# ZhonghuaYi/EI-Nexus_official

Measured on AMD Instinct MI355X. Metric: event-image pairs/s (extract+match, 346x260, 1024 kpts), higher is better.
Workload: dtype f32; 1 GPU; B32 346x260 5-bin event voxel + gray image, VGG(event)+SuperPoint(image) extractors, MNN matcher, k=1024; global_batch=32, event_bins=5, parallelism=dp1 (pairs sharded, metric all-reduce only), log_assignment=False, dense_outputs=False, same_scene_pairs=False, weights=seeded synthetic, descriptor-head bias calibrated (per-channel mean removed)

## Files before the change

### ei-nexus_official_amd/_lib.py

```python
import ctypes
import os

_HERE = os.path.dirname(os.path.abspath(__file__))
LIB_PATH = os.environ.get("EINX_LIB") or os.path.join(_HERE, "libeinx_hip.so")

c_void_p, c_int, c_float, c_size_t, c_char_p = ctypes.c_void_p, ctypes.c_int, ctypes.c_float, ctypes.c_size_t, ctypes.c_char_p


class ConvDesc(ctypes.Structure):
    _fields_ = [("w_native", c_void_p), ("bias", c_void_p), ("scale", c_void_p), ("shift", c_void_p),
                ("cin", ctypes.c_int32), ("cout", ctypes.c_int32), ("ks", ctypes.c_int32), ("relu", ctypes.c_int32),
                ("pool", ctypes.c_int32)]


class DetectParams(ctypes.Structure):
    _fields_ = [("B", ctypes.c_int32), ("Hp", ctypes.c_int32), ("Wp", ctypes.c_int32), ("H", ctypes.c_int32),
                ("W", ctypes.c_int32), ("h0", ctypes.c_int32), ("w0", ctypes.c_int32), ("radius", ctypes.c_int32),
                ("top_k", ctypes.c_int32), ("det_thr", c_float), ("ordering_xy", ctypes.c_int32), ("cap", ctypes.c_int32),
                ("nms_iters", ctypes.c_int32)]


class ExtractorDesc(ctypes.Structure):
    _fields_ = [("struct_size", c_size_t), ("cell", ctypes.c_int32), ("n_backbone", ctypes.c_int32), ("n_det", ctypes.c_int32), ("n_desc", ctypes.c_int32),
                ("backbone", ctypes.POINTER(ConvDesc)), ("det_head", ctypes.POINTER(ConvDesc)), ("desc_head", ctypes.POINTER(ConvDesc)),
# ... 41 lines not shown
                ("t_type", ctypes.c_int32), ("p_type", ctypes.c_int32), ("n", ctypes.c_int64)]


class LgLayer(ctypes.Structure):
    _names = ("Wqkv", "bqkv", "Wo", "bo", "sf0_w", "sf0_b", "sln_g", "sln_b", "sf3_w", "sf3_b",
              "Wqk", "bqk", "Wv", "bv", "Wco", "bco", "cf0_w", "cf0_b", "cln_g", "cln_b", "cf3_w", "cf3_b", "Wqk_v", "bqk_v")
    _fields_ = [(n, c_void_p) for n in _names]


class LgWeights(ctypes.Structure):
    _fields_ = [("struct_size", c_size_t), ("layer_size", c_size_t), ("in_w", c_void_p), ("in_b", c_void_p), ("Wr", c_void_p), ("proj_w", c_void_p), ("proj_b", c_void_p),
                ("match_w", c_void_p), ("match_b", c_void_p), ("n_layers", ctypes.c_int32), ("heads", ctypes.c_int32),
                ("d", ctypes.c_int32), ("input_dim", ctypes.c_int32), ("filter_threshold", c_float),
                ("layers", ctypes.POINTER(LgLayer))]


class LgHead(ctypes.Structure):
    _fields_ = [(n, c_void_p) for n in ("proj_w", "proj_b", "match_w", "match_b", "token_w", "token_b")]


SIGNATURES = {
    "einx_version": (c_char_p, []),
    "einx_abi_version": (c_int, []),
    "einx_build_flags": (c_char_p, []),
    "einx_params_hash": (c_int, [c_void_p, c_int, c_void_p, c_void_p, c_void_p, c_void_p]),
    "einx_last_error": (c_char_p, []),
    "einx_math_eval": (c_int, [c_int, c_void_p, ctypes.c_longlong, c_void_p, c_void_p]),
    "einx_fork_stream_of": (c_void_p, [c_void_p]),
    "einx_fork_stream_prepare_beside": (c_int, [c_void_p, ctypes.POINTER(c_void_p), c_int]),
    "einx_stream_overlap_us": (c_int, [c_void_p, c_void_p, c_int, ctypes.POINTER(ctypes.c_float)]),
    "einx_device_count": (c_int, []),
    "einx_profile_enable": (c_int, [c_int]),
    "einx_profile_report": (c_int, [c_char_p, c_size_t]),
    "einx_extractor_create": (c_void_p, [ctypes.POINTER(ExtractorDesc)]),
    "einx_extractor_destroy": (None, [c_void_p]),
    "einx_fork_stream_prepare": (c_int, [c_void_p]),
    "einx_fork_stream_release": (c_int, [c_void_p]),
    "einx_fork_stream_count": (c_int, []),
    "einx_side_stream": (c_void_p, [c_void_p, c_int, ctypes.POINTER(c_void_p), c_int]),
    "einx_extract_shapes": (c_int, [c_void_p, c_int, c_int, ctypes.POINTER(ExtractShapes)]),
    "einx_extract_ws_bytes": (c_size_t, [c_void_p, c_int, c_int, c_int, c_int, c_int]),
    "einx_extract": (c_int, [c_void_p, c_void_p, c_void_p, c_int, c_int, c_int, c_int, c_void_p, c_size_t, ctypes.POINTER(ExtractOut), c_void_p]),
    "einx_extract_watch": (c_int, [c_void_p, c_void_p, c_void_p, c_int, c_int, c_int, c_int, c_void_p, c_size_t, ctypes.POINTER(ExtractOut),
                           ctypes.POINTER(WeightWatch), c_void_p]),
    "einx_conv_last_kernel": (c_char_p, []),
    "einx_conv_plan": (c_char_p, [c_int] * 11),
    "einx_conv_weight_elems": (c_size_t, [c_int, c_int, c_int]),
    "einx_conv_repack": (c_int, [c_void_p, c_int, c_int, c_int, c_void_p, c_void_p]),
    "einx_bn_fold": (c_int, [c_void_p, c_void_p, c_void_p, c_void_p, c_float, c_int, c_void_p, c_void_p, c_void_p]),
    "einx_conv_block": (c_int, [c_void_p, c_int, c_int, c_int, c_int, c_int, c_int, c_int, ctypes.POINTER(ConvDesc), c_void_p, c_void_p]),
    "einx_conv_first_two_fused_ok": (c_int, [ctypes.POINTER(ConvDesc), ctypes.POINTER(ConvDesc), c_int, c_int, c_int]),
    "einx_conv_first_two_fused": (c_int, [c_void_p, c_int, c_int, c_int, c_int, c_int, c_int, c_int, ctypes.POINTER(ConvDesc), ctypes.POINTER(ConvDesc),
                                  c_void_p, c_void_p]),
    "einx_div_inplace": (c_int, [c_void_p, c_size_t, c_float, c_void_p]),
    "einx_image_prepare": (c_int, [c_void_p, c_int, c_int, c_int, c_int, ctypes.c_longlong, ctypes.c_longlong, ctypes.c_longlong, ctypes.c_longlong,
                           c_float, c_void_p, c_void_p]),
    "einx_score_map": (c_int, [c_void_p, c_int, c_int, c_int, c_int, c_void_p, c_int, c_int, c_int, c_int, c_int, c_int, c_void_p,
                               c_void_p, c_void_p]),
    "einx_remove_border": (c_int, [c_void_p, c_int, c_int, c_int, c_int, c_void_p]),
    "einx_detect_ws_bytes": (c_size_t, [ctypes.POINTER(DetectParams)]),
    "einx_detect": (c_int, [c_void_p, ctypes.POINTER(DetectParams), c_void_p, c_void_p, c_void_p, c_void_p, c_void_p, c_void_p,
                            c_void_p, c_void_p]),
    "einx_desc_sample": (c_int, [c_void_p, c_int, c_int, c_int, c_int, c_int, c_int, c_int, c_int, c_void_p, c_void_p, c_int, c_float,
                                 c_void_p, c_void_p]),
    "einx_normalize_map": (c_int, [c_void_p, c_int, c_int, c_int, c_float, c_void_p, c_void_p, c_void_p]),
    "einx_upsample_ws_bytes": (c_size_t, [c_int, c_int, c_int]),
    "einx_upsample_normalize": (c_int, [c_void_p, c_int, c_int, c_int, c_int, c_int, c_int, c_int, c_int, c_int, c_int, c_float,
                                        c_void_p, c_void_p, c_size_t, c_void_p]),
    "einx_mnn_ws_bytes": (c_size_t, [c_int, c_int, c_int]),
    "einx_mnn": (c_int, [c_void_p, c_void_p, c_int, c_void_p, c_void_p, c_int, c_int, c_int, c_void_p, c_void_p, c_void_p, c_void_p,
                         c_void_p, c_void_p, c_void_p]),
    "einx_mnn_gather": (c_int, [c_void_p, c_void_p, c_int, c_void_p, c_void_p, c_int, c_int, c_int, c_void_p, c_void_p, c_void_p, c_void_p,
                                c_void_p, c_void_p, c_void_p, c_void_p, c_int, c_void_p, c_void_p, c_void_p, c_void_p]),
    "einx_mnn_thresh": (c_int, [c_void_p, c_void_p, c_int, c_void_p, c_void_p, c_int, c_int, c_int, c_int, c_float, c_int, c_float, c_void_p,
                                c_void_p, c_void_p, c_void_p, c_void_p, c_void_p, c_void_p]),
    "einx_gather_matches": (c_int, [c_void_p, c_void_p, c_void_p, c_void_p, c_int, c_int, c_int, c_int, c_void_p, c_void_p, c_void_p,
                                    c_void_p]),
    "einx_events_ws_bytes": (c_size_t, [c_int, c_int, c_int]),
    "einx_voxel_ws_bytes": (c_size_t, [c_int, c_int, c_int, c_int, ctypes.c_int64]),
    "einx_voxel_grid": (c_int, [c_void_p, c_void_p, c_void_p, c_void_p, c_void_p, c_int, c_int, c_int, c_int, c_int, c_void_p, c_void_p,
                                c_size_t, c_void_p]),
    "einx_events_mask": (c_int, [c_void_p, c_void_p, c_void_p, c_int, c_int, c_int, c_void_p, c_void_p, c_void_p]),
    "einx_time_surface_ws_bytes": (c_size_t, [c_int, c_int, c_int, c_int, ctypes.c_int64]),
    "einx_event_stack_ws_bytes": (c_size_t, [c_int, c_int, c_int, c_int, ctypes.c_int64]),
    "einx_distance_map_ws_bytes": (c_size_t, [c_int, c_int, c_int, c_int, ctypes.c_int64]),
    "einx_time_surface": (c_int, [c_void_p, c_void_p, c_void_p, c_void_p, c_void_p, c_int, c_int, c_int, c_int, c_void_p, c_void_p, c_size_t,
                                  c_void_p]),
    "einx_event_stack": (c_int, [c_void_p, c_void_p, c_void_p, c_void_p, c_void_p, c_int, c_int, c_int, c_int, c_void_p, c_void_p, c_size_t,
                                 c_void_p]),
    "einx_distance_map": (c_int, [c_void_p, c_void_p, c_void_p, c_void_p, c_void_p, c_int, c_int, c_int, c_int, c_void_p, c_void_p, c_size_t,
                                  c_void_p]),
    "einx_distance_map_plan": (c_char_p, [c_int, c_int]),
    "einx_events_windows_ws_bytes": (c_size_t, [c_int, c_int, c_int]),
    "einx_voxel_windows_ws_bytes": (c_size_t, [c_int, c_int, c_int, c_int, ctypes.c_int64]),
    "einx_voxel_grid_windows": (c_int, [c_void_p, c_void_p, c_void_p, c_void_p, ctypes.c_int64, c_void_p, c_void_p, c_int, c_int, c_int, c_int, c_int,
                                        c_void_p, c_void_p, c_size_t, c_void_p]),
    "einx_events_mask_windows": (c_int, [c_void_p, c_void_p, ctypes.c_int64, c_void_p, c_void_p, c_int, c_int, c_int, c_void_p, c_size_t, c_void_p,
                                         c_void_p]),
    "einx_events_pack": (c_int, [ctypes.POINTER(EventArrays), c_int, c_void_p, c_void_p, c_void_p, c_void_p, c_void_p, c_int]),
    "einx_metrics_ws_bytes": (c_size_t, [ctypes.POINTER(MetricParams)]),
    "einx_pair_metrics": (c_int, [ctypes.POINTER(MetricParams)] + [c_void_p] * 13),
    "einx_relative_pose_ws_bytes": (c_size_t, [ctypes.POINTER(PoseParams)]),
    "einx_relative_pose": (c_int, [ctypes.POINTER(PoseParams)] + [c_void_p] * 13),
    "einx_essential_5pt": (c_int, [c_void_p, c_void_p, c_int, c_void_p, c_void_p, c_void_p]),
    "einx_homography_ws_bytes": (c_size_t, [ctypes.POINTER(HomographyParams)]),
    "einx_homography": (c_int, [ctypes.POINTER(HomographyParams)] + [c_void_p] * 11),
# ... 67 lines not shown
```

### ei-nexus_official_amd/csrc/conv.hip

```cpp
#include <stdio.h>
#include <stdlib.h>

#include <type_traits>

#include "einx_common.h"

namespace {

constexpr int kCoutTile = 64;

struct ConvArgs {
  const float* in;
  const float* w;
  const float* bias;
  const float* scale;
  const float* shift;
  float* out;
  int B, Cin, Cout, CoutPad;
  int Hs, Ws, h0, w0;
  int H, W;
  int tilesX, tilesY;
  int relu;
};

// ... 819 lines not shown
    const float* ib = in_b + (size_t)c * CK * HW;
#pragma unroll
    for (int i = 0; i < IN_PER_THR; ++i) r_in[i] = ib[goff[i]];
    const float* wb = a.w + (size_t)c * CK * a.CoutPad;
#pragma unroll
    for (int i = 0; i < W_PER_THR; ++i) r_w[i] = *reinterpret_cast<const f32x4*>(wb + woff[i]);
  };
  f32x4v acc[NPW];
#pragma unroll
  for (int n = 0; n < NPW; ++n) acc[n] = f32x4v{0.0f, 0.0f, 0.0f, 0.0f};
  const int nchunks = a.Cin / CK;
  issue_loads(0);
  float e_bi[4], e_sc[4], e_sh[4];
#pragma unroll
  for (int i = 0; i < 4; ++i) {
    const int coc = min(co0 + wave * 16 + 4 * q + i, a.Cout - 1);
    e_bi[i] = a.bias ? a.bias[coc] : 0.0f;
    e_sc[i] = a.scale ? a.scale[coc] : 1.0f;
    e_sh[i] = a.scale ? a.shift[coc] : 0.0f;
  }
  const int aoff = q * WP + wave * 16 + j, boff = q * NPX + j;
  for (int c = 0; c < nchunks; ++c) {
    __syncthreads();
#pragma unroll
    for (int i = 0; i < IN_PER_THR; ++i) in_tile[loff[i]] = r_in[i];
#pragma unroll
    for (int i = 0; i < W_PER_THR; ++i) *reinterpret_cast<f32x4*>(w_tile + wl[i]) = r_w[i];
    __syncthreads();
    if (c + 1 < nchunks) issue_loads(c + 1);
    float av[G], bv[G][NPW];
#pragma unroll
    for (int g = 0; g < G; ++g) {
      av[g] = w_tile[aoff + g * 4 * WP];
#pragma unroll
      for (int n = 0; n < NPW; ++n) bv[g][n] = in_tile[boff + g * 4 * NPX + 16 * n];
    }
#pragma unroll
    for (int g = 0; g < G; ++g)
#pragma unroll
      for (int n = 0; n < NPW; ++n) acc[n] = __builtin_amdgcn_mfma_f32_16x16x4f32(av[g], bv[g][n], acc[n], 0, 0, 0);
  }
  float* out_b = a.out + (size_t)b * a.Cout * HW;
#pragma unroll
  for (int i = 0; i < 4; ++i) {
    const int co = co0 + wave * 16 + 4 * q + i;
#pragma unroll
    for (int n = 0; n < NPW; ++n) {
      const int p = p0 + 16 * n + j;
      float v = acc[n][i] + e_bi[i];
      if (a.relu) v = v > 0.0f ? v : 0.0f;
      if (a.scale) v = fmaf(v, e_sc[i], e_sh[i]);
      if (co < a.Cout && p < HW) out_b[(size_t)co * HW + p] = v;
    }
  }
}

__global__ void conv_repack_kernel(const float* w, int cin, int cout, int taps, int coutPad, int krows, float* out) {
  const size_t n = (size_t)krows * coutPad;
  for (size_t i = (size_t)blockIdx.x * blockDim.x + threadIdx.x; i < n; i += (size_t)gridDim.x * blockDim.x) {
    const int co = (int)(i % coutPad);
    const int k = (int)(i / coutPad);
    const int h = k & 1;
    const int tap = (k >> 1) % taps;
    const int cp = (k >> 1) / taps;
    const int ci = 2 * cp + h;
    float v = 0.0f;
    if (ci < cin && co < cout) v = w[((size_t)co * cin + ci) * taps + tap];
    out[i] = v;
  }
}

__global__ void bn_fold_kernel(const float* g, const float* b, const float* mean, const float* var, float eps, int n, float* scale,
                               float* shift) {
  const int i = blockIdx.x * blockDim.x + threadIdx.x;
  if (i >= n) return;
  const float s = g[i] / sqrtf(var[i] + eps);
  scale[i] = s;
  shift[i] = b[i] - mean[i] * s;
}

int native_krows(int cin, int taps) { return einx_cdiv(cin, 32) * 32 * taps; }

thread_local const char* g_last_conv_kernel = "";

struct TileCfg {
  int th, tw, slots;
};

template <int KS, int TH, int TW, int WM, int WN, int MT, int NT, int CK, bool POOL, bool DENSE3 = false>
void launch(const ConvArgs& a, int B, hipStream_t s, bool three_per_cu = false) {
  dim3 grid((unsigned)(a.tilesX * a.tilesY * B), (unsigned)(a.CoutPad / kCoutTile));
  const bool three = DENSE3 && three_per_cu;
  {
    static char nm[2][96] = {{0}, {0}};
    char* n = nm[three ? 1 : 0];
    if (!n[0]) snprintf(n, sizeof nm[0], "conv_block_kernel<%d,%d,%d,%d,%d,%d,%d,%d,%s>%s", KS, TH, TW, WM, WN, MT, NT, CK, POOL ? "true" : "false", three ? " (3 per CU)" : "");
    g_last_conv_kernel = n;
  }
  EINX_PROF(KS == 1 ? "conv_block_kernel 1x1" : (CK < 8 ? "conv_block_kernel 3x3 first layer" : "conv_block_kernel 3x3"), s);
  if constexpr (DENSE3) {
    if (three) {
      hipLaunchKernelGGL((conv_block_kernel<KS, TH, TW, WM, WN, MT, NT, CK, POOL, false, 6>), grid, dim3(WM * WN * 64), 0, s, a);
      return;
    }
  }
  hipLaunchKernelGGL((conv_block_kernel<KS, TH, TW, WM, WN, MT, NT, CK, POOL>), grid, dim3(WM * WN * 64), 0, s, a);
// ... 336 lines not shown
    EINX_CONV_BLOCK_VARIANTS(X)
#undef X
    case CB_1X1_128_XTRA: {
      dim3 grid((unsigned)(a.tilesX * B), (unsigned)(a.CoutPad / kCoutTile - 1));
      conv_plan_name(p, d->pool, nm, sizeof nm);
      g_last_conv_kernel = nm;
      EINX_PROF("conv_block_kernel 1x1", s);
      hipLaunchKernelGGL((conv_block_kernel<1, 1, 128, 1, 4, 2, 1, 32, false, true>), grid, dim3(256), 0, s, a);
      break;
    }
    case C16_1X1: {
      dim3 grid((unsigned)(a.tilesX * B), (unsigned)(a.CoutPad / kCoutTile));
      conv_plan_name(p, d->pool, nm, sizeof nm);
      g_last_conv_kernel = nm;
      EINX_PROF("conv16_1x1_kernel (small grid)", s);
      if (p.npw == 4) hipLaunchKernelGGL(conv16_1x1_kernel<4>, grid, dim3(256), 0, s, a);
      else if (p.npw == 2) hipLaunchKernelGGL(conv16_1x1_kernel<2>, grid, dim3(256), 0, s, a);
      else hipLaunchKernelGGL(conv16_1x1_kernel<1>, grid, dim3(256), 0, s, a);
      break;
    }
    default: {
      dim3 grid((unsigned)(a.tilesX * a.tilesY * B), (unsigned)(a.CoutPad / kCoutTile));
      conv_plan_name(p, d->pool, nm, sizeof nm);
      g_last_conv_kernel = nm;
      EINX_PROF("conv16_kernel 3x3 (small grid)", s);
#define EINX_C16(P, N) hipLaunchKernelGGL((conv16_kernel<P, 8, N>), grid, dim3(256), 0, s, a)
      if (d->pool) {
        if (p.npw == 4) EINX_C16(true, 4);
        else if (p.npw == 2) EINX_C16(true, 2);
        else EINX_C16(true, 1);
      } else {
        if (p.npw == 4) EINX_C16(false, 4);
        else if (p.npw == 2) EINX_C16(false, 2);
        else EINX_C16(false, 1);
      }
#undef EINX_C16
      break;
    }
  }
  EINX_CHECK_LAUNCH();
  return EINX_OK;
}

EINX_EXPORT const char* einx_conv_plan(int cin, int cout, int ks, int pool, int B, int Hs, int Ws, int h0, int w0, int H, int W) {
  const ConvPlanLayer pl = {cin, cout, ks, pool};
  if (const char* refused = conv_shape_refused(&pl, B, Hs, Ws, h0, w0, H, W)) {
    einx_set_error("%s: %s", __func__, refused);
    return nullptr;
  }
  static thread_local char nm[96];
  conv_plan_name(conv_plan(&pl, B, Hs, Ws, h0, w0, H, W), pool, nm, sizeof nm);
  return nm;
}
```

### ei-nexus_official_amd/csrc/extract.hip

```cpp
#include <stdlib.h>
#include <string.h>

#include <algorithm>
#include <mutex>
#include <new>
#include <vector>

#include "einx_common.h"

struct einx_extractor {
  einx_extractor_desc d;
  std::vector<einx_conv_desc> backbone, det, desc;
  bool has_merged = false;
  einx_conv_desc merged;
};

namespace {

struct Plan {
  int Hp, Wp, h0, w0;
  int hc, wc;
  size_t buf_elems[2];
  size_t head_elems;
};

constexpr long kForkMaxCells = 8192;
bool fork_heads(const einx_extractor* e, const Plan& pl, int B) { return e->d.cell == 8 || (long)B * pl.hc * pl.wc <= kForkMaxCells; }

void padder(int h, int w, int p, int* w0, int* w1, int* h0, int* h1) {
  const int hp = (((h / p) + 1) * p - h) % p;
  const int wp = (((w / p) + 1) * p - w) % p;
  *w0 = wp / 2;
  *w1 = wp - wp / 2;
  *h0 = hp / 2;
  *h1 = hp - hp / 2;
}

bool make_plan(const einx_extractor* e, int H, int W, Plan* pl) {
  int w0, w1, h0, h1;
  padder(H, W, e->d.cell, &w0, &w1, &h0, &h1);
  pl->Hp = H + h0 + h1;
  pl->Wp = W + w0 + w1;
  pl->h0 = h0;
  pl->w0 = w0;
  int h = pl->Hp, w = pl->Wp;
  pl->buf_elems[0] = pl->buf_elems[1] = 0;
  const int nb = (int)e->backbone.size();
  for (int i = 0; i < nb; ++i) {
    const einx_conv_desc& c = e->backbone[i];
    if (c.pool) {
      if ((h & 1) || (w & 1)) return false;
      h /= 2;
      w /= 2;
    }
    if (i + 1 < nb) {
      const size_t n = (size_t)c.cout * h * w;
      if (n > pl->buf_elems[i & 1]) pl->buf_elems[i & 1] = n;
    }
  }
  pl->hc = h;
  pl->wc = w;
  size_t he = 0;
  for (size_t i = 0; i + 1 < e->det.size(); ++i) he = std::max(he, (size_t)e->det[i].cout * h * w);
  for (size_t i = 0; i + 1 < e->desc.size(); ++i) he = std::max(he, (size_t)e->desc[i].cout * h * w);
  if (e->has_merged) he = std::max(he, (size_t)e->merged.cout * h * w);
  pl->head_elems = he;
  return h * e->d.cell == pl->Hp && w * e->d.cell == pl->Wp;
}

int topk_cap(int N, int top_k, float det_thr) {
  if (top_k <= 0 || top_k >= N || det_thr < 1.0f) return N;
  const float q = (float)(N - top_k) / (float)N;
  const float rank = q * (float)(N - 1);
  const int lo = (int)floorf(rank);
  return N - 1 - lo;
}

void detect_params(const einx_extractor* e, const Plan& pl, int B, int H, int W, int cap, int nms_iters, einx_detect_params* p) {
  p->B = B;
  p->Hp = pl.Hp;
  p->Wp = pl.Wp;
  p->H = H;
  p->W = W;
  p->h0 = pl.h0;
  p->w0 = pl.w0;
  p->radius = e->d.nms_radius;
  p->top_k = e->d.top_k;
  p->det_thr = e->d.det_thr;
  p->ordering_xy = e->d.ordering_xy;
  p->cap = cap;
  p->nms_iters = nms_iters;
}

}

EINX_EXPORT einx_extractor* einx_extractor_create(const einx_extractor_desc* d) {
  if (!d) {
    einx_set_error("einx_extractor_create: null descriptor");
    return nullptr;
  }
  if (d->struct_size != sizeof(einx_extractor_desc)) {
    einx_set_error("einx_extractor_create: einx_extractor_desc::struct_size is %zu, this library's is %zu (header / library ABI mismatch: EINX_ABI_VERSION %d)",
                   (size_t)d->struct_size, sizeof(einx_extractor_desc), EINX_ABI_VERSION);
    return nullptr;
  }
  if (!d || !d->backbone || !d->det_head || !d->desc_head || d->n_backbone <= 0 || d->n_det <= 0 || d->n_desc <= 0) {
    einx_set_error("einx_extractor_create: null / empty layer lists");
    return nullptr;
  }
  if (d->cell != 8 && d->cell != 1) {
    einx_set_error("einx_extractor_create: cell must be 8 (SuperPoint-shaped) or 1 (SiLK-shaped)");
    return nullptr;
  }
  einx_extractor* e = new (std::nothrow) einx_extractor();
  if (!e) return nullptr;
  e->d = *d;
  e->backbone.assign(d->backbone, d->backbone + d->n_backbone);
  e->det.assign(d->det_head, d->det_head + d->n_det);
  e->desc.assign(d->desc_head, d->desc_head + d->n_desc);
  e->d.backbone = e->backbone.data();
  e->d.det_head = e->det.data();
  e->d.desc_head = e->desc.data();
  e->d.merged_head0 = nullptr;
  if (d->merged_head0) {
    const einx_conv_desc& m = *d->merged_head0;
    const einx_conv_desc &a = e->det.front(), &b = e->desc.front();
    if (e->det.size() != 2 || e->desc.size() != 2 || m.cin != a.cin || m.cin != b.cin || m.cout != a.cout + b.cout || m.ks != a.ks || m.ks != b.ks ||
        m.relu != a.relu || m.relu != b.relu || m.pool || a.pool || b.pool || !m.w_native || (m.scale == nullptr) != (a.scale == nullptr) ||
// ... 70 lines not shown
}

EINX_EXPORT int einx_extract(const einx_extractor* e, float* in, const uint8_t* mask, int B, int H, int W, int nms_iters, void* ws,
                             size_t ws_bytes, const einx_extract_out* o, void* stream) {
  return einx_extract_watch(e, in, mask, B, H, W, nms_iters, ws, ws_bytes, o, nullptr, stream);
}

EINX_EXPORT int einx_extract_watch(const einx_extractor* e, float* in, const uint8_t* mask, int B, int H, int W, int nms_iters, void* ws,
                                   size_t ws_bytes, const einx_extract_out* o, const einx_weight_watch* ww, void* stream) {
  EINX_CHECK_ARG(e && in && ws && o, "null pointer");
  EINX_CHECK_ARG(!ww || ww->struct_size == sizeof(einx_weight_watch), "einx_weight_watch::struct_size does not match this library (ABI mismatch)");
  EINX_CHECK_ARG(!ww || ww->n == 0 || (ww->n > 0 && ww->table && ww->ref && ww->scratch && ww->stale), "weight watch with null pointers");
  EINX_CHECK_ARG(o->feats && o->logits && o->raw && o->prob && o->score && o->positions && o->indices && o->counts && o->thr &&
                     o->not_converged && o->sparse_desc,
                 "null output pointer");
  EINX_CHECK_ARG(B > 0 && H > 0 && W > 0 && o->cap > 0, "bad shape");
  Plan pl;
  EINX_CHECK_ARG(make_plan(e, H, W, &pl), "image size does not fit the network's pooling / cell size");
  EINX_CHECK_ARG(e->d.cell == 1 || (o->coarse && o->raw_cl), "cell-8 networks need the coarse / raw_cl outputs");
  EINX_CHECK_ARG(ws_bytes >= einx_extract_ws_bytes(e, B, H, W, o->cap, nms_iters), "workspace smaller than einx_extract_ws_bytes for these arguments");
  einx_detect_params dp;
  detect_params(e, pl, B, H, W, o->cap, nms_budget(nms_iters), &dp);
  WsCarver c{(char*)ws};
  const ExtractWs wk = carve(c, e, pl, &dp, B);
  bool fork = fork_heads(e, pl, B) && !einx_profile_active();
  {
    hipStreamCaptureStatus cs = hipStreamCaptureStatusNone;
    if (fork && hipStreamIsCapturing((hipStream_t)stream, &cs) == hipSuccess && cs != hipStreamCaptureStatusNone) fork = false;
  }
  float* const head2 = fork ? wk.head2 : wk.head;
  int rc;
  if (e->d.input_div != 0.0f && e->d.input_div != 1.0f) {
    rc = einx_div_inplace(in, (size_t)B * e->backbone.front().cin * H * W, e->d.input_div, stream);
    if (rc) return rc;
  }
  const float* cur = in;
  int h = pl.Hp, w = pl.Wp;
  const int nb = (int)e->backbone.size();
  int first = 0;
  if (nb >= 2 && 1 == einx_conv_first_two_fused_ok(&e->backbone[0], &e->backbone[1], B, pl.Hp, pl.Wp)) {
    float* out = (2 < nb) ? wk.buf[1] : o->feats;
    if ((rc = einx_conv_first_two_fused(in, B, H, W, pl.h0, pl.w0, pl.Hp, pl.Wp, &e->backbone[0], &e->backbone[1], out, stream))) return rc;
    if (e->backbone[1].pool) {
      h /= 2;
      w /= 2;
    }
    cur = out;
    first = 2;
  }
  for (int i = first; i < nb; ++i) {
    const einx_conv_desc& c = e->backbone[i];
    float* out = (i + 1 < nb) ? wk.buf[i & 1] : o->feats;
    if (i == 0) rc = einx_conv_block(cur, B, H, W, pl.h0, pl.w0, pl.Hp, pl.Wp, &c, out, stream);
    else rc = einx_conv_block(cur, B, h, w, 0, 0, h, w, &c, out, stream);
    if (rc) return rc;
    if (c.pool) {
      h /= 2;
      w /= 2;
    }
    cur = out;
  }
  auto run_head = [&](const std::vector<einx_conv_desc>& L, float* scratch, float* final_out, void* st) -> int {
    const float* x = o->feats;
    for (size_t i = 0; i < L.size(); ++i) {
      float* out = (i + 1 < L.size()) ? scratch : final_out;
      const int r = einx_conv_block(x, B, h, w, 0, 0, h, w, &L[i], out, st);
      if (r) return r;
      x = out;
    }
    return 0;
  };
  const int D = e->desc.back().cout;
  const bool merged = e->has_merged && B == 1;
  if (merged && (rc = einx_conv_block(o->feats, B, h, w, 0, 0, h, w, &e->merged, wk.head, stream))) return rc;
  const float* desc_in = wk.head + (size_t)e->det.front().cout * h * w;
  auto det_branch = [&](void* st) -> int {
    if (merged) return einx_conv_block(wk.head, B, h, w, 0, 0, h, w, &e->det[1], o->logits, st);
    return run_head(e->det, wk.head, o->logits, st);
  };
  auto desc_branch = [&](void* st) -> int {
    int r = merged ? einx_conv_block(desc_in, B, h, w, 0, 0, h, w, &e->desc[1], o->raw, st) : run_head(e->desc, head2, o->raw, st);
    if (r) return r;
    if (e->d.cell == 8) r = einx_normalize_map(o->raw, B, D, h * w, e->d.desc_scale, o->coarse, o->raw_cl, st);
    return r;
  };
  std::unique_lock<std::mutex> side_lock;
  const EinxSide* sd = fork ? einx_side_acquire((hipStream_t)stream, &side_lock) : nullptr;
  if (sd) {
    if (hipEventRecord(sd->fork, (hipStream_t)stream) != hipSuccess || hipStreamWaitEvent(sd->stream, sd->fork, 0) != hipSuccess) {
      einx_set_error("einx_extract: fork failed");
      return EINX_ERR_LAUNCH;
    }
    rc = desc_branch(sd->stream);
    const bool ok = hipEventRecord(sd->join, sd->stream) == hipSuccess;
    if (rc) {
      (void)hipStreamWaitEvent((hipStream_t)stream, sd->join, 0);
      return rc;
    }
    if (!ok) {
      einx_set_error("einx_extract: join failed");
      return EINX_ERR_LAUNCH;
    }
    if ((rc = det_branch(stream))) {
      (void)hipStreamWaitEvent((hipStream_t)stream, sd->join, 0);
      return rc;
    }
  } else {
    if ((rc = det_branch(stream))) return rc;
    if ((rc = desc_branch(stream))) return rc;
  }
  const int C_det = e->det.back().cout;
  const long score_threads = (long)(C_det == 65 ? einx_cdiv(B * h * w, 32) : einx_cdiv(B * h * w, 256)) * 256;
  const bool zero_in_score = wk.det.nflags > 0 && wk.det.nflags <= score_threads;
  rc = einx_score_map_zero(o->logits, B, C_det, h, w, mask, H, W, pl.h0, pl.w0, e->d.dilate_mask, e->d.border, o->prob, o->score,
                           zero_in_score ? wk.det.flags : nullptr, zero_in_score ? wk.det.nflags : 0, o->score_crop, stream);
  if (rc) {
    if (sd) (void)hipStreamWaitEvent((hipStream_t)stream, sd->join, 0);
    return rc;
  }
// ... 32 lines not shown
```

### include/einx.h

```cpp
#ifndef EINX_H
#define EINX_H

#include <stddef.h>
#include <stdint.h>

#ifdef __cplusplus
extern "C" {
#endif

#define EINX_OK 0
#define EINX_ERR_ARG (-1)
#define EINX_ERR_LAUNCH (-2)
#define EINX_ERR_NO_DEVICE (-3)

#define EINX_ABI_VERSION 6
int einx_abi_version(void);
const char* einx_version(void);
const char* einx_last_error(void);
const char* einx_build_flags(void);
int einx_device_count(void);

#define EINX_WATCH_CHUNK_WORDS 4096
int einx_params_hash(const int64_t* table, int n, uint64_t* hash, const uint64_t* ref, int32_t* stale, void* stream);

int einx_math_eval(int fn, const float* x, long long n, float* y, void* stream);

int einx_stream_overlap_us(void* stream_a, void* stream_b, int spin_us, float* elapsed_us);

int einx_profile_enable(int on);
int einx_profile_report(char* buf, size_t cap);


size_t einx_conv_weight_elems(int cin, int cout, int ks);
int einx_conv_repack(const float* w_oihw, int cin, int cout, int ks, float* w_native, void* stream);

int einx_bn_fold(const float* gamma, const float* beta, const float* mean, const float* var, float eps, int n, float* scale,
                 float* shift, void* stream);

typedef struct einx_conv_desc {
  const float* w_native;
  const float* bias;
  const float* scale;
  const float* shift;
  int32_t cin, cout, ks;
  int32_t relu;
  int32_t pool;
} einx_conv_desc;

int einx_conv_block(const float* in, int B, int Hs, int Ws, int h0, int w0, int H, int W, const einx_conv_desc* d, float* out,
                    void* stream);

int einx_conv_first_two_fused_ok(const einx_conv_desc* d0, const einx_conv_desc* d1, int B, int H, int W);
int einx_conv_first_two_fused(const float* in, int B, int Hs, int Ws, int h0, int w0, int H, int W, const einx_conv_desc* d0,
                              const einx_conv_desc* d1, float* out, void* stream);

const char* einx_conv_last_kernel(void);

const char* einx_conv_plan(int cin, int cout, int ks, int pool, int B, int Hs, int Ws, int h0, int w0, int H, int W);

int einx_div_inplace(float* x, size_t n, float divisor, void* stream);

int einx_image_prepare(float* image, int B, int C, int H, int W, long long stride_b, long long stride_c, long long stride_h,
                       long long stride_w, float divisor, float* gray, void* stream);


int einx_score_map(const float* logits, int B, int C, int hc, int wc, const uint8_t* mask, int H, int W, int h0, int w0,
                   int dilate, int border, float* prob, float* score, void* stream);

int einx_remove_border(float* score, int B, int Hp, int Wp, int border, void* stream);

int einx_dense_positions(const float* score, int B, int H, int W, int ordering_xy, float* out, void* stream);

typedef struct einx_detect_params {
  int32_t B, Hp, Wp;
  int32_t H, W, h0, w0;
  int32_t radius;
  int32_t top_k;
  float det_thr;
  int32_t ordering_xy;
  int32_t cap;
  int32_t nms_iters;
} einx_detect_params;

size_t einx_detect_ws_bytes(const einx_detect_params* p);

int einx_detect(const float* score, const einx_detect_params* p, void* ws, float* nms_out, float* positions, int32_t* indices,
                int32_t* counts, float* thr, int32_t* not_converged, void* stream);


int einx_desc_sample(const float* raw, int B, int D, int hc, int wc, int Hp, int Wp, int bilinear, int channels_last,
                     const int32_t* indices, const int32_t* counts, int cap, float scale, float* out, void* stream);

int einx_normalize_map(const float* raw, int B, int D, int P, float scale, float* out, float* raw_cl, void* stream);

int einx_normalize_rows(const float* x, int R, int C, float scale, float* out, void* stream);

int einx_random_positions(const float* u, int R, float size0, float size1, float* out, void* stream);

size_t einx_upsample_ws_bytes(int B, int H, int W);
int einx_upsample_normalize(const float* raw, int B, int D, int hc, int wc, int Hp, int Wp, int h0, int w0, int H, int W,
                            float scale, float* out, void* ws, size_t ws_bytes, void* stream);

size_t einx_mnn_ws_bytes(int B, int cap0, int cap1);
int einx_mnn(const float* desc0, const int32_t* n, int cap0, const float* desc1, const int32_t* m, int cap1, int B, int D,
             void* ws, int64_t* matches0, int64_t* matches1, float* scores0, float* scores1, float* la, void* stream);
int einx_mnn_gather(const float* desc0, const int32_t* n, int cap0, const float* desc1, const int32_t* m, int cap1, int B, int D,
                    void* ws, int64_t* matches0, int64_t* matches1, float* scores0, float* scores1, float* la, const float* kpts0,
// ... 262 lines not shown
```

Measured before the change: 3787 pairs/s.

## Add 22x8-tile 3x3 conv kernel with fused pooling for small feature maps

Adds a new MFMA 3x3 convolution kernel using 22x8 pixel tiles, a bank-conflict-free LDS layout chosen at compile time, register-prefetched input and weight chunks, and 2x2 max-pooling fused into the epilogue via lane shuffles. A dispatcher routes pooling layers whose spatial shape divides into 22-row tiles (and is not covered by existing tile shapes) to it. The aim is better tile fit and occupancy on odd-sized maps such as 66-row feature maps, where the existing tilings waste work. It adds a specialised code path used for few layers.

```diff
diff --git a/ei-nexus_official_amd/_lib.py b/ei-nexus_official_amd/_lib.py
--- a/ei-nexus_official_amd/_lib.py
+++ b/ei-nexus_official_amd/_lib.py
@@ -117,6 +117,9 @@
     "einx_conv_first_two_fused_ok": (c_int, [ctypes.POINTER(ConvDesc), ctypes.POINTER(ConvDesc), c_int, c_int, c_int]),
     "einx_conv_first_two_fused": (c_int, [c_void_p, c_int, c_int, c_int, c_int, c_int, c_int, c_int, ctypes.POINTER(ConvDesc), ctypes.POINTER(ConvDesc),
                                   c_void_p, c_void_p]),
+    "einx_conv_block_px16_ok": (c_int, [ctypes.POINTER(ConvDesc), c_int, c_int, c_int, c_int, c_int, c_int, c_int]),
+    "einx_conv_block_px16": (c_int, [c_void_p, c_int, c_int, c_int, c_int, c_int, c_int, c_int, ctypes.POINTER(ConvDesc), c_int, c_int,
+                             c_void_p, c_void_p]),
     "einx_div_inplace": (c_int, [c_void_p, c_size_t, c_float, c_void_p]),
     "einx_image_prepare": (c_int, [c_void_p, c_int, c_int, c_int, c_int, ctypes.c_longlong, ctypes.c_longlong, ctypes.c_longlong, ctypes.c_longlong,
                            c_float, c_void_p, c_void_p]),
diff --git a/ei-nexus_official_amd/csrc/conv.hip b/ei-nexus_official_amd/csrc/conv.hip
--- a/ei-nexus_official_amd/csrc/conv.hip
+++ b/ei-nexus_official_amd/csrc/conv.hip
@@ -895,6 +895,234 @@
       if (a.scale) v = fmaf(v, e_sc[i], e_sh[i]);
       if (co < a.Cout && p < HW) out_b[(size_t)co * HW + p] = v;
     }
+  }
+}
+
+struct Px16Lds {
+  int pitch, plane;
+};
+constexpr bool px16_conflict_free(int th, int tw, int pitch, int plane) {
+  for (int t = 0; t < th * tw / 16; ++t) {
+    unsigned used = 0;
+    for (int h = 0; h < 2; ++h)
+      for (int j = 0; j < 16; ++j) {
+        const int q = 16 * t + j;
+        const unsigned bit = 1u << ((h * plane + (q / tw) * pitch + q % tw) & 31);
+        if (used & bit) return false;
+        used |= bit;
+      }
+  }
+  return true;
+}
+constexpr Px16Lds px16_lds(int th, int tw) {
+  Px16Lds best = {tw + 2, (th + 2) * (tw + 2)};
+  bool found = false;
+  for (int p = tw + 2; p < tw + 2 + 32; ++p)
+    for (int pad = 0; pad < 32; ++pad) {
+      const int plane = (th + 2) * p + pad;
+      if ((!found || plane < best.plane) && px16_conflict_free(th, tw, p, plane)) {
+        best = {p, plane};
+        found = true;
+      }
+    }
+  return best;
+}
+
+template <int TH, int TW, bool POOL>
+__global__ __launch_bounds__(256, 4) void conv_px16_kernel(const ConvArgs a) {
+  constexpr int CK = 8, TAPS = 9, KCH = CK * TAPS, G = KCH / 4;
+  constexpr int NTHR = 256;
+  constexpr int PW = TW + 2, PH = TH + 2;
+  constexpr Px16Lds LAY = px16_lds(TH, TW);
+  constexpr int PITCH = LAY.pitch, PLANE = LAY.plane;
+  constexpr int PLANE_E = PH * PW;
+  constexpr int NPIX = TH * TW;
+  constexpr int TROWS = 16 / TW;
+  constexpr int NA = NPIX / 16;
+  static_assert(TW == 8 && TH % TROWS == 0, "an N-tile is two rows of 8 pixels");
+  static_assert(!POOL || TH % 2 == 0, "every 2x2 window lives inside one tile");
+  static_assert(px16_conflict_free(TH, TW, PITCH, PLANE), "no conflict-free LDS layout");
+  static_assert(PLANE_E <= NTHR, "one staging thread per halo position");
+  constexpr int NG = conv_stage_groups(NTHR, PLANE_E, CK);
+  constexpr int CPT = CK / NG;
+  constexpr int WP = kCoutTile + 16;
+  constexpr int W_F4 = KCH * kCoutTile / 4;
+  constexpr int W_PER_THR = (W_F4 + NTHR - 1) / NTHR;
+  static_assert(NTHR % (kCoutTile / 4) == 0, "a thread's weight float4s sit a whole number of rows apart");
+  __shared__ __attribute__((aligned(16))) float in_tile[CK * PLANE];
+  __shared__ __attribute__((aligned(16))) float w_tile[KCH * WP];
+  __shared__ __attribute__((aligned(16))) float s_bias[kCoutTile], s_scale[kCoutTile], s_shift[kCoutTile];
+
+  const int tid = threadIdx.x;
+  const int wave = __builtin_amdgcn_readfirstlane(tid >> 6);
+  const int wm = wave;
+  const int lane = tid & 63;
+  const int q = lane >> 4, j = lane & 15;
+
+  const int ncot = (int)gridDim.y;
+  int item = xcd_contiguous((int)(blockIdx.x + blockIdx.y * gridDim.x), (int)gridDim.x * ncot);
+  const int co0 = (item % ncot) * kCoutTile;
+  int bid = item / ncot;
+  const int tx_i = bid % a.tilesX;
+  bid /= a.tilesX;
+  const int ty_i = bid % a.tilesY;
+  const int b = bid / a.tilesY;
+  if (tid < kCoutTile) {
+    const int co = co0 + tid;
+    const bool cv = co < a.Cout;
+    s_bias[tid] = (cv && a.bias) ? a.bias[co] : 0.0f;
+    s_scale[tid] = (cv && a.scale) ? a.scale[co] : 1.0f;
+    s_shift[tid] = (cv && a.scale) ? a.shift[co] : 0.0f;
+  }
+  const int y0 = ty_i * TH, x0 = tx_i * TW;
+
+  const int jy = j >> 3, jx = j & 7;
+  const int bpix = (q & 1) * PLANE + jy * PITCH + jx;
+  const int up = q >> 1;
+  const int bB[3] = {bpix + up, bpix + up * (PITCH - 2), bpix + up * (2 * PLANE - 2 * PITCH - 2)};
+  const int aB = q * WP + wm * 16 + j;
+
+  const unsigned src_plane = (unsigned)(a.H * a.W);
+  const float* in_b = a.in + (size_t)b * a.Cin * src_plane;
+  const int pos = NG == 1 ? tid : tid % PLANE_E;
+  const int grp = NG == 1 ? 0 : tid / PLANE_E;
+  const bool s_active = NG * PLANE_E == NTHR || tid < NG * PLANE_E;
+  int src_off = -1;
+  {
+    const int py = pos / PW, px = pos % PW;
+    const int y = y0 - 1 + py, x = x0 - 1 + px;
+    if (y >= 0 && y < a.H && x >= 0 && x < a.W) src_off = y * a.W + x;
+  }
+  const int lds_pos = grp * CPT * PLANE + (pos / PW) * PITCH + pos % PW;
+  const bool s_ok = s_active && src_off >= 0;
+  const unsigned in_voff = ((unsigned)(src_off >= 0 ? src_off : 0) + (unsigned)(grp * CPT) * src_plane) * 4u;
+  if (s_active && src_off < 0) {
+#pragma unroll
+    for (int i = 0; i < CPT; ++i) in_tile[lds_pos + i * PLANE] = 0.0f;
+  }
+  const unsigned woff = (unsigned)((tid / (kCoutTile / 4)) * a.CoutPad + co0 + (tid % (kCoutTile / 4)) * 4) * 4u;
+  const unsigned wstep = (unsigned)((NTHR / (kCoutTile / 4)) * a.CoutPad) * 4u;
+  const int wl = (tid / (kCoutTile / 4)) * WP + (tid % (kCoutTile / 4)) * 4;
+
+  f32x4v acc[NA];
+#pragma unroll
+  for (int n = 0; n < NA; ++n) acc[n] = f32x4v{0.0f, 0.0f, 0.0f, 0.0f};
+
+  const int nchunks = a.Cin / CK;
+  float r_in[CPT];
+  f32x4 r_w[W_PER_THR];
+  auto issue_loads = [&](int c) {
+    const int ci0 = c * CK;
+    if (s_ok) {
+      const __amdgpu_buffer_rsrc_t rs = conv_rsrc(in_b + (size_t)ci0 * src_plane, (unsigned)(a.Cin - ci0) * src_plane * 4u);
+#pragma unroll
+      for (int i = 0; i < CPT; ++i)
+        r_in[i] = __builtin_bit_cast(float, __builtin_amdgcn_raw_buffer_load_b32(rs, in_voff, (unsigned)i * src_plane * 4u, 0));
+    }
+    const __amdgpu_buffer_rsrc_t rw = conv_rsrc(a.w + (size_t)c * KCH * a.CoutPad, (unsigned)(KCH * a.CoutPad) * 4u);
+#pragma unroll
+    for (int i = 0; i < W_PER_THR; ++i)
+      if ((i + 1) * NTHR <= W_F4 || tid + i * NTHR < W_F4)
+        r_w[i] = __builtin_bit_cast(f32x4, __builtin_amdgcn_raw_buffer_load_b128(rw, woff, (unsigned)i * wstep, 0));
+  };
+  auto commit_loads = [&]() {
+    if (s_ok) {
+#pragma unroll
+      for (int i = 0; i < CPT; ++i) in_tile[lds_pos + i * PLANE] = r_in[i];
+    }
+#pragma unroll
+    for (int i = 0; i < W_PER_THR; ++i)
+      if ((i + 1) * NTHR <= W_F4 || tid + i * NTHR < W_F4) *reinterpret_cast<f32x4*>(w_tile + wl + i * (NTHR / (kCoutTile / 4)) * WP) = r_w[i];
+  };
+  auto mfma_chunk = [&]() {
+    float av[2], bv[2][NA];
+    auto load_frag = [&](int g, int buf) {
+      const int s = 2 * g, pair = s / TAPS, tap = s % TAPS;
+      const int kind = tap == TAPS - 1 ? 2 : (tap % 3 == 2 ? 1 : 0);
+      const int off = pair * 2 * PLANE + (tap / 3) * PITCH + tap % 3;
+      av[buf] = w_tile[aB + g * 4 * WP];
+#pragma unroll
+      for (int n = 0; n < NA; ++n) bv[buf][n] = in_tile[bB[kind] + off + n * TROWS * PITCH];
+    };
+    load_frag(0, 0);
+#pragma unroll
+    for (int g = 0; g < G; ++g) {
+      if (g + 1 < G) load_frag(g + 1, (g + 1) & 1);
+      __builtin_amdgcn_sched_barrier(0);
+#pragma unroll
+      for (int n = 0; n < NA; ++n) acc[n] = __builtin_amdgcn_mfma_f32_16x16x4f32(av[g & 1], bv[g & 1][n], acc[n], 0, 0, 0);
+      __builtin_amdgcn_sched_barrier(0);
+    }
+  };
+  issue_loads(0);
+  for (int c = 0; c < nchunks; ++c) {
+    __syncthreads();
+    commit_loads();
+    __syncthreads();
+    if (c + 1 < nchunks) issue_loads(c + 1);
+    mfma_chunk();
+  }
+
+  const int Ho = POOL ? a.H / 2 : a.H, Wo = POOL ? a.W / 2 : a.W;
+  const unsigned plane_o = (unsigned)(Ho * Wo);
+  float* out_b = a.out + (size_t)b * a.Cout * plane_o;
+  unsigned ovoff[NA];
+#pragma unroll
+  for (int o = 0; o < NA; ++o) {
+    const int ty = o * TROWS + jy, tx = jx;
+    const int y = y0 + ty, x = x0 + tx;
+    int pix = -1;
+    if (POOL) {
+      const int yo = y >> 1, xo = x >> 1;
+      if (!(ty & 1) && !(tx & 1) && yo < Ho && xo < Wo) pix = yo * Wo + xo;
+    } else {
+      if (y < a.H && x < a.W) pix = y * a.W + x;
+    }
+    ovoff[o] = pix >= 0 ? ((unsigned)pix + (unsigned)(4 * q) * plane_o) * 4u : 0xFFFFFFFFu;
+  }
+  auto epilogue = [&](auto relu_c, auto aff_c) {
+    constexpr bool RELU = decltype(relu_c)::value, AFF = decltype(aff_c)::value;
+    const int cl0 = wm * 16;
+    const f32x4 bi = *reinterpret_cast<const f32x4*>(&s_bias[cl0 + 4 * q]);
+    f32x4 sc, sh;
+    if (AFF) {
+      sc = *reinterpret_cast<const f32x4*>(&s_scale[cl0 + 4 * q]);
+      sh = *reinterpret_cast<const f32x4*>(&s_shift[cl0 + 4 * q]);
+    }
+#pragma unroll
+    for (int i = 0; i < 4; ++i) {
+      const int co_r = co0 + cl0 + i;
+      const int nch = a.Cout - co_r > 0 ? a.Cout - co_r : 0;
+      const __amdgpu_buffer_rsrc_t ro = conv_rsrc(out_b + (size_t)co_r * plane_o, (unsigned)nch * plane_o * 4u);
+      float pv[NA];
+#pragma unroll
+      for (int n = 0; n < NA; ++n) {
+        float v = acc[n][i] + bi[i];
+        if (RELU) v = fmaxf(v, 0.0f);
+        if (AFF) v = fmaf(v, sc[i], sh[i]);
+        pv[n] = v;
+      }
+      if (!POOL) {
+#pragma unroll
+        for (int n = 0; n < NA; ++n) __builtin_amdgcn_raw_buffer_store_b32(__builtin_bit_cast(unsigned, pv[n]), ro, ovoff[n], 0, 0);
+      } else {
+#pragma unroll
+        for (int n = 0; n < NA; ++n) {
+          float m = max_lane_xor<8>(pv[n]);
+          m = max_lane_xor<1>(m);
+          __builtin_amdgcn_raw_buffer_store_b32(__builtin_bit_cast(unsigned, m), ro, ovoff[n], 0, 0);
+        }
+      }
+    }
+  };
+  using T_ = std::integral_constant<bool, true>;
+  using F_ = std::integral_constant<bool, false>;
+  if (a.relu) {
+    if (a.scale) epilogue(T_{}, T_{});
+    else epilogue(T_{}, F_{});
+  } else {
+    if (a.scale) epilogue(F_{}, T_{});
+    else epilogue(F_{}, F_{});
   }
 }
 
@@ -1337,3 +1565,70 @@
   conv_plan_name(conv_plan(&pl, B, Hs, Ws, h0, w0, H, W), pool, nm, sizeof nm);
   return nm;
 }
+
+namespace {
+
+constexpr long kPx16MinWorkgroups = 512;
+
+const char* px16_refused(const einx_conv_desc* d, int B, int Hs, int Ws, int h0, int w0, int H, int W) {
+  if (d->ks != 3) return "3x3 layers only";
+  const ConvPlanLayer pl = {d->cin, d->cout, d->ks, d->pool};
+  if (const char* r = conv_shape_refused(&pl, B, Hs, Ws, h0, w0, H, W)) return r;
+  if (Hs != H || Ws != W || h0 != 0 || w0 != 0) return "no replicate-pad fold";
+  if (d->cin % 8 != 0) return "input channels must be a multiple of 8";
+  return nullptr;
+}
+
+template <int TH, int TW>
+void launch_px16(const ConvArgs& a, int B, bool pool, hipStream_t s) {
+  dim3 grid((unsigned)(a.tilesX * a.tilesY * B), (unsigned)(a.CoutPad / kCoutTile));
+  static char nm[2][64] = {{0}, {0}};
+  char* n = nm[pool ? 1 : 0];
+  if (!n[0]) snprintf(n, sizeof nm[0], "conv_px16_kernel<%d,%d,%s>", TH, TW, pool ? "true" : "false");
+  g_last_conv_kernel = n;
+  EINX_PROF("conv_block_kernel px16 3x3", s);
+  if (pool) hipLaunchKernelGGL((conv_px16_kernel<TH, TW, true>), grid, dim3(256), 0, s, a);
+  else hipLaunchKernelGGL((conv_px16_kernel<TH, TW, false>), grid, dim3(256), 0, s, a);
+}
+
+}
+
+EINX_EXPORT int einx_conv_block_px16_ok(const einx_conv_desc* d, int B, int Hs, int Ws, int h0, int w0, int H, int W) {
+  if (!d || px16_refused(d, B, Hs, Ws, h0, w0, H, W)) return 0;
+  if (!d->pool) return 0;
+  if ((H % 12 == 0 && W % 16 == 0) || (H % 8 == 0 && W % 32 == 0)) return 0;
+  if (H % 22 == 0 && W % 8 == 0 && (long)(H / 22) * (W / 8) * B * einx_cdiv(d->cout, kCoutTile) >= kPx16MinWorkgroups) return 1;
+  return 0;
+}
+
+EINX_EXPORT int einx_conv_block_px16(const float* in, int B, int Hs, int Ws, int h0, int w0, int H, int W, const einx_conv_desc* d, int th,
+                                     int tw, float* out, void* stream) {
+  EINX_CHECK_ARG(in && out && d && d->w_native, "null pointer");
+  EINX_CHECK_ARG((d->scale == nullptr) == (d->shift == nullptr), "scale and shift go together");
+  const char* refused = px16_refused(d, B, Hs, Ws, h0, w0, H, W);
+  EINX_CHECK_ARG(!refused, refused);
+  EINX_CHECK_ARG(th == 22 && tw == 8, "tile must be 22x8");
+  ConvArgs a;
+  a.in = in;
+  a.w = d->w_native;
+  a.bias = d->bias;
+  a.scale = d->scale;
+  a.shift = d->shift;
+  a.out = out;
+  a.B = B;
+  a.Cin = d->cin;
+  a.Cout = d->cout;
+  a.CoutPad = einx_cdiv(d->cout, kCoutTile) * kCoutTile;
+  a.Hs = H;
+  a.Ws = W;
+  a.h0 = 0;
+  a.w0 = 0;
+  a.H = H;
+  a.W = W;
+  a.relu = d->relu;
+  a.tilesX = einx_cdiv(W, tw);
+  a.tilesY = einx_cdiv(H, th);
+  launch_px16<22, 8>(a, B, d->pool != 0, (hipStream_t)stream);
+  EINX_CHECK_LAUNCH();
+  return EINX_OK;
+}
diff --git a/ei-nexus_official_amd/csrc/extract.hip b/ei-nexus_official_amd/csrc/extract.hip
--- a/ei-nexus_official_amd/csrc/extract.hip
+++ b/ei-nexus_official_amd/csrc/extract.hip
@@ -74,6 +74,11 @@
   const float rank = q * (float)(N - 1);
   const int lo = (int)floorf(rank);
   return N - 1 - lo;
+}
+
+int conv_layer(const float* x, int B, int h, int w, const einx_conv_desc* c, float* out, void* stream) {
+  if (einx_conv_block_px16_ok(c, B, h, w, 0, 0, h, w) == 1) return einx_conv_block_px16(x, B, h, w, 0, 0, h, w, c, 22, 8, out, stream);
+  return einx_conv_block(x, B, h, w, 0, 0, h, w, c, out, stream);
 }
 
 void detect_params(const einx_extractor* e, const Plan& pl, int B, int H, int W, int cap, int nms_iters, einx_detect_params* p) {
@@ -250,7 +255,7 @@
     const einx_conv_desc& c = e->backbone[i];
     float* out = (i + 1 < nb) ? wk.buf[i & 1] : o->feats;
     if (i == 0) rc = einx_conv_block(cur, B, H, W, pl.h0, pl.w0, pl.Hp, pl.Wp, &c, out, stream);
-    else rc = einx_conv_block(cur, B, h, w, 0, 0, h, w, &c, out, stream);
+    else rc = conv_layer(cur, B, h, w, &c, out, stream);
     if (rc) return rc;
     if (c.pool) {
       h /= 2;
@@ -262,7 +267,7 @@
     const float* x = o->feats;
     for (size_t i = 0; i < L.size(); ++i) {
       float* out = (i + 1 < L.size()) ? scratch : final_out;
-      const int r = einx_conv_block(x, B, h, w, 0, 0, h, w, &L[i], out, st);
+      const int r = conv_layer(x, B, h, w, &L[i], out, st);
       if (r) return r;
       x = out;
     }
diff --git a/include/einx.h b/include/einx.h
--- a/include/einx.h
+++ b/include/einx.h
@@ -53,6 +53,10 @@
 int einx_conv_first_two_fused_ok(const einx_conv_desc* d0, const einx_conv_desc* d1, int B, int H, int W);
 int einx_conv_first_two_fused(const float* in, int B, int Hs, int Ws, int h0, int w0, int H, int W, const einx_conv_desc* d0,
                               const einx_conv_desc* d1, float* out, void* stream);
+
+int einx_conv_block_px16_ok(const einx_conv_desc* d, int B, int Hs, int Ws, int h0, int w0, int H, int W);
+int einx_conv_block_px16(const float* in, int B, int Hs, int Ws, int h0, int w0, int H, int W, const einx_conv_desc* d, int th, int tw,
+                         float* out, void* stream);
 
 const char* einx_conv_last_kernel(void);
 
```

Measured after the change: 3805 pairs/s (median of 2 runs). About the same (+0.5%).
